# RFD-FHEM/PySignalduino

Hardware: AMD Instinct MI355X
Metric: RF messages/sec demodulated (MU+MS+MC, full protocol bank) (higher is better)
Workload: dtype u8+f64; 1 GPU; mixed MU/MS/MC stream, 1/3 each per rank: MU 256-pulse messages x 129-id MU bank, MS sync+bits x 66-id MS bank (clock x U(0.6,1.4)), MC frames x 12 clockrange ids ('fixed' chain); kind=mixed, corpus=bench, msgs_per_gpu=1000000, batches=3, input_bytes_resident=571611860, parallelism=dp1, grouped=True, streams=one kernel (k_step: MU, then MS, then MC tiles)

## Files before the change

pysignalduino_amd/csrc/sdx_device.h:

```cpp
#pragma once
#include <hip/hip_runtime.h>
#include <stdint.h>

#include "../../include/sdx.h"
#include "../../include/sdx_bank.h"

#define SDX_DEV __device__ __forceinline__

namespace sdx {

constexpr int WAVE = 64;

SDX_DEV double py_round1(double q) {
  if (!(fabs(q) < 562949953421312.0)) return q;
  double f = floor(q * 10.0);
  if (fma(10.0, q, -f) < 0.0) f -= 1.0;
  else if (fma(10.0, q, -(f + 1.0)) >= 0.0) f += 1.0;
  const double r = fma(10.0, q, -(f + 0.5));
  double k;
  if (r > 0.0) k = f + 1.0;
  else if (r < 0.0) k = f;
  else k = (((long long)f & 1) == 0) ? f : f + 1.0;
  double res = k / 10.0;
  if (res == 0.0) res = copysign(0.0, q);
  return res;
}

constexpr int SDX_K_NONE = INT32_MIN;
SDX_DEV int py_round1_k(double q) {
  if (!(fabs(q) < 67108864.0)) return SDX_K_NONE;
  double f = floor(q * 10.0);
  if (fma(10.0, q, -f) < 0.0) f -= 1.0;
  else if (fma(10.0, q, -(f + 1.0)) >= 0.0) f += 1.0;
  const double r = fma(10.0, q, -(f + 0.5));
  double k;
  if (r > 0.0) k = f + 1.0;
  else if (r < 0.0) k = f;
  else k = (((long long)f & 1) == 0) ? f : f + 1.0;
  return (int)k;
}
SDX_DEV void sort10(uint32_t* a) {
#define SDX_CE(i, j)                      \
  {                                       \
    const uint32_t x = a[i], y = a[j];    \
    a[i] = x < y ? x : y;                 \
    a[j] = x < y ? y : x;                 \
  }
  SDX_CE(4, 9) SDX_CE(3, 8) SDX_CE(2, 7) SDX_CE(1, 6) SDX_CE(0, 5) SDX_CE(1, 4) SDX_CE(6, 9) SDX_CE(0, 3)
  SDX_CE(5, 8) SDX_CE(0, 2) SDX_CE(3, 6) SDX_CE(7, 9) SDX_CE(0, 1) SDX_CE(2, 4) SDX_CE(5, 7) SDX_CE(8, 9)
  SDX_CE(1, 2) SDX_CE(4, 6) SDX_CE(7, 8) SDX_CE(3, 5) SDX_CE(2, 5) SDX_CE(6, 8) SDX_CE(1, 3) SDX_CE(4, 7)
  SDX_CE(2, 3) SDX_CE(6, 7) SDX_CE(3, 4) SDX_CE(5, 6) SDX_CE(4, 5)
#undef SDX_CE
}

SDX_DEV bool k_in(int k, int klo, int khi) { return (uint32_t)k - (uint32_t)klo <= (uint32_t)khi - (uint32_t)klo; }

SDX_DEV int lane_id() { return __lane_id(); }
SDX_DEV uint64_t ballot(bool p) { return __ballot(p); }
SDX_DEV int bcast_i(int v, int src) { return __shfl(v, src); }
SDX_DEV uint64_t bcast_u64(uint64_t v, int src) {
  uint32_t lo = __shfl((uint32_t)v, src), hi = __shfl((uint32_t)(v >> 32), src);
  return ((uint64_t)hi << 32) | lo;
}
SDX_DEV int ffs64(uint64_t x) { return __ffsll((unsigned long long)x) - 1; }
SDX_DEV int popc64(uint64_t x) { return __popcll(x); }

SDX_DEV uint64_t bm_window(const uint64_t* bm, int w, int sh, int nw) {
  uint64_t lo = bm[w];
  if (sh == 0) return lo;
  uint64_t hi = (w + 1 < nw) ? bm[w + 1] : 0ull;
  return (lo >> sh) | (hi << (64 - sh));
}

struct PexRes {
  bool found;
  int pos;
  uint64_t tgt;
};

SDX_DEV bool substr_first(const uint64_t* bm, int ws, int nw, uint64_t tgt, int tlen, int minpos, int* pos) {
  for (int w = minpos >> 6; w < nw; ++w) {
    uint64_t acc = ~0ull;
    for (int i = 0; i < tlen && acc; ++i) {
      const int id = (int)((tgt >> (4 * i)) & 15);
      const int sh = i & 63, wo = w + (i >> 6);
      uint64_t v = 0;
      if (wo < nw) v = bm_window(bm + id * ws, wo, sh, nw);
      acc &= v;
    }
    if (w == (minpos >> 6) && (minpos & 63)) acc &= ~0ull << (minpos & 63);
    if (acc) {
      *pos = w * 64 + ffs64(acc);
      return true;
    }
  }
  return false;
}

__device__ __noinline__ PexRes pattern_exists(const sdx_patspec* sp, const int* kq, uint64_t ids, int npat,
                                              const uint64_t* bm, int ws, int nw, int minpos) {
  PexRes res{false, -1, 0};
  const int nu = sp->nuniq, slen = sp->len;
  uint64_t cand[SDX_MAXUNIQ];
  int cnt[SDX_MAXUNIQ];
  long long total = 1;
#pragma unroll
  for (int u = 0; u < SDX_MAXUNIQ; ++u) {
    cand[u] = 0;
    cnt[u] = 1;
    if (u < nu) {
      const double v = sp->uval[u];
      const int klo = sp->klo[u], khi = sp->khi[u];
      double gap[SDX_MAXPAT];
      bool ok[SDX_MAXPAT];
#pragma unroll
      for (int j = 0; j < SDX_MAXPAT; ++j) {
        ok[j] = (j < npat) && k_in(kq[j], klo, khi);
        gap[j] = fabs((double)kq[j] / 10.0 - v);
      }
      int c = 0;
      uint64_t packed = 0;
#pragma unroll
      for (int j = 0; j < SDX_MAXPAT; ++j) {
        if (ok[j]) {
          int rank = 0;
#pragma unroll
          for (int k = 0; k < SDX_MAXPAT; ++k)
            rank += (ok[k] && (gap[k] < gap[j] || (gap[k] == gap[j] && k < j))) ? 1 : 0;
          packed |= (uint64_t)j << (4 * rank);
          ++c;
        }
      }
      cand[u] = packed;
      cnt[u] = c;
      total *= c;
      if (total > 10000) total = 10001;
    }
  }
  if (nu == 0) return res;
  for (int u = 0; u < nu; ++u)
    if (cnt[u] == 0) return res;
  if (total > 10000) return res;
  int digit[SDX_MAXUNIQ];
#pragma unroll
  for (int u = 0; u < SDX_MAXUNIQ; ++u) digit[u] = 0;
  for (long long it = 0; it < total; ++it) {
    uint32_t used = 0, uid = 0;
    bool dup = false;
#pragma unroll
    for (int u = 0; u < SDX_MAXUNIQ; ++u) {
      if (u < nu) {
        const int slot = (int)((cand[u] >> (4 * digit[u])) & 15);
        if (used & (1u << slot)) dup = true;
        used |= 1u << slot;
        uid |= (uint32_t)((ids >> (4 * slot)) & 15) << (4 * u);
      }
    }
    if (!dup) {
      uint64_t tgt = 0;
      for (int i = 0; i < slen; ++i) tgt |= (uint64_t)((uid >> (4 * sp->uidx[i])) & 15) << (4 * i);
      int pos;
      if (substr_first(bm, ws, nw, tgt, slen, minpos, &pos)) {
        res.found = true;
        res.pos = pos;
        res.tgt = tgt;
        return res;
      }
    }
#pragma unroll
    for (int u = SDX_MAXUNIQ - 1; u >= 0; --u) {
      if (u < nu) {
        if (digit[u] + 1 < cnt[u]) {
          digit[u]++;
          break;
        }
        digit[u] = 0;
      }
    }
  }
  return res;
}

SDX_DEV bool match_at(const uint64_t* bm, int ws, int n, uint64_t tgt, int tlen, int x) {
  if (x < 0 || x + tlen > n) return false;
  for (int i = 0; i < tlen; ++i) {
    const int id = (int)((tgt >> (4 * i)) & 15), p = x + i;
    if (!((bm[id * ws + (p >> 6)] >> (p & 63)) & 1ull)) return false;
  }
  return true;
}

SDX_DEV int bval(const uint8_t* b, int a, int e) {
  int v = 0;
  for (int i = a; i < e; ++i) v = (v << 1) | b[i];
  return v;
}
SDX_DEV int first_one(const uint8_t* b, int n) {
  for (int i = 0; i < n; ++i)
    if (b[i] == 1) return i;
  return -1;
}

SDX_DEV int pd_em(const uint8_t* b, int n, uint8_t* o, int* no) {
  int p = -1;
  for (int i = 0; i + 10 <= n; ++i) {
    bool ok = b[i + 9] == 1;
    for (int j = 0; ok && j < 9; ++j) ok = b[i + j] == 0;
    if (ok) { p = i; break; }
  }
  if (p < 0) return 0;
  const uint8_t* s = b + p + 10;
  const int m = n - p - 10;
  if (m != 89) return 0;
  int crc = 0, k = 0;
  for (int c = 0; c + 8 < m; c += 9) {
    if (c < m - 10) {
      for (int j = 7; j >= 0; --j) o[k++] = s[c + j];
      crc ^= bval(s, c, c + 8);
    }
  }
  if (crc != bval(s, m - 8, m)) return 0;
  *no = k;
  return 1;
}

SDX_DEV int pd_revolt(const uint8_t* b, int n, uint8_t* o, int* no) {
  if (n < 96) return 0;
  int sum = 0;
  for (int i = 0; i < 88; i += 8) sum += bval(b, i, i + 8);
  if ((sum & 0xFF) != bval(b, 88, 96)) return 0;
  for (int i = 0; i < 88; ++i) o[i] = b[i];
  *no = 88;
  return 1;
}

SDX_DEV bool groups9_even(const uint8_t* m, int k) {
  for (int g = 0; g < k; g += 9) {
    int par = 0;
    for (int i = g; i < g + 9 && i < k; ++i) par += m[i];
    if (par & 1) return false;
  }
  return true;
}

SDX_DEV int pd_fs20(const uint8_t* b, int n, uint8_t* o, int* no) {
  const int st = first_one(b, n);
  if (st < 0) return 0;
  const uint8_t* m = b + st + 1;
  int k = n - st - 1;
  if (k == 46 || k == 55) --k;
  if (k != 45 && k != 54) return 0;
  int sum = 6;
  for (int g = 0; g < k - 9; g += 9) sum += bval(m, g, g + 8);
  const int chk = bval(m, k - 9, k - 1);
  if (((sum + 6) & 0xFF) == chk) return 0;
  if ((sum & 0xFF) != chk) return 0;
  if (!groups9_even(m, k)) return 0;
  const int nbytes = k / 9;
  int q = 0;
  for (int g = 0; g < nbytes; ++g) {
    if (k == 45 && g == 3) for (int j = 0; j < 8; ++j) o[q++] = 0;
    if (g == nbytes - 1) break;
    for (int j = 0; j < 8; ++j) o[q++] = m[9 * g + j];
  }
  *no = q;
  return 1;
}

SDX_DEV int pd_fht80(const uint8_t* b, int n, uint8_t* o, int* no) {
  const int st = first_one(b, n);
  if (st < 0) return 0;
  const uint8_t* m = b + st + 1;
  int k = n - st - 1;
  if (k == 55) --k;
  if (k != 54) return 0;
  int sum = 12;
  for (int g = 0; g < 45; g += 9) sum += bval(m, g, g + 8);
  const int chk = bval(m, 45, 53);
  if (((sum - 6) & 0xFF) == chk) return 0;
  if ((sum & 0xFF) != chk) return 0;
  if (!groups9_even(m, 54)) return 0;
  int q = 0;
  for (int g = 0; g < 6; ++g)
    for (int j = 0; j < 8; ++j) o[q++] = m[9 * g + j];
  *no = q;
  return 1;
}

SDX_DEV int pd_fht80tf(const uint8_t* b, int n, uint8_t* o, int* no) {
  if (n < 46) return 0;
  const int st = first_one(b, n);
  if (st < 0) return 0;
  const uint8_t* m = b + st + 1;
  const int k = n - st - 1;
  if (k != 45) return 0;
  int sum = 12;
  for (int g = 0; g < 36; g += 9) sum += bval(m, g, g + 8);
  if ((sum & 0xFF) != bval(m, 36, 44)) return 0;
  if (!groups9_even(m, 45)) return 0;
  if (m[9 * 3 + 2] != 0) return 0;
  int q = 0;
  for (int g = 0; g < 4; ++g)
    for (int j = 0; j < 8; ++j) o[q++] = m[9 * g + j];
  *no = q;
  return 1;
}

SDX_DEV int rev_nib(const uint8_t* b, int a, int e) {
  int v = 0;
  for (int i = e - 1; i >= a; --i) v = (v << 1) | b[i];
  return v;
}
SDX_DEV int pd_ws2000(const uint8_t* b, int n, uint8_t* o, int* no) {
  const int st = first_one(b, n);
  if (st < 0) return 0;
  const int dlen = n - st;
  int dlen1 = dlen - dlen % 5;
  const int te = (st + 5 < n) ? st + 5 : n;
  if (te <= st + 1) return -1;
  const int typ = rev_nib(b, st + 1, te);
  if (typ > 7) return 0;
  if (typ == 1 && (dlen == 45 || dlen == 46)) dlen1 += 5;
  const int tab[8] = {35, 50, 35, 50, 70, 40, 40, 85};
  if (tab[typ] != dlen1) return 0;
  if (st > 10) return 0;
  int idx = 0, didx = 0, check = 0, acc = 5;
  while (idx < dlen - 1) {
    if (b[idx + st] != 1) return 0;
    didx = idx + st + 1;
    if (n - didx < 4) return 0;
    const int nib = rev_nib(b, didx, didx + 4);
    if (dlen == 45 || dlen == 46) {
      if (idx <= dlen - 5) check ^= nib;
    } else if (idx <= dlen - 10) {
      check ^= nib;
      acc += nib;
    }
    idx += 5;
  }
  if (check != 0) return 0;
  if (dlen < 45 || dlen > 46) {
    const int e = (didx + 4 < n) ? didx + 4 : n;
    if (e <= didx) return -1;
    if (rev_nib(b, didx, e) != (acc & 0x0F)) return 0;
  }
  const int d = st + 1;
  int q = 0;
  auto rv = [&](int a, int e) {
    for (int i = d + e - 1; i >= d + a; --i)
      if (i < n) o[q++] = b[i];
  };
  rv(5, 9); rv(0, 4); rv(15, 19); rv(10, 14);
  if (typ == 0 || typ == 2) {
    rv(20, 24);
  } else if (typ == 1 || typ == 3 || typ == 4 || typ == 7) {
    rv(25, 29); rv(20, 24); rv(35, 39); rv(30, 34);
    if (typ == 4) { rv(55, 59); rv(50, 54); rv(45, 49); rv(40, 44); }
  }
  *no = q;
  return 1;
}

SDX_DEV int pd_ws7035(const uint8_t* b, int n, uint8_t* o, int* no) {
  if (n < 8) return 0;
  const uint8_t ident[8] = {1, 0, 1, 0, 0, 0, 0, 0};
  for (int i = 0; i < 8; ++i)
    if (b[i] != ident[i]) return 0;
  if (n != 44) return 0;
// ... 148 lines not shown
```

pysignalduino_amd/csrc/sdx_group.hip:

```cpp
#include "sdx_device.h"
#include "sdx_lane.h"

namespace sdx {

SDX_DEV int lanes_below_mask(uint64_t mask) {
  const int l = lane_id();
  return popc64(l ? (mask & ((1ull << l) - 1)) : 0ull);
}
SDX_DEV uint64_t peers8(uint32_t v, bool active) {
  uint64_t peers = ballot(active);
#pragma unroll
  for (int bit = 0; bit < 8; ++bit) {
    const uint64_t bb = ballot(active && ((v >> bit) & 1u));
    peers &= ((v >> bit) & 1u) ? bb : ~bb;
  }
  return peers;
}

constexpr int SIG_PROTOS = 32;
template <int KIND>
SDX_DEV void sig_block(const void* __restrict__ bank, const sdx_pulse_batch& b, uint32_t* __restrict__ key,
                       uint32_t* __restrict__ msg_out, sdx_msg_rec* __restrict__ mrec, const int blk) {
  const BankView bv = bank_view(bank);
  const int i = blk * 256 + threadIdx.x;
  const int ntot = b.sel_dev ? b.n_sel : b.n;
  const bool valid = i < ntot;
  const int msg = valid ? (b.sel_dev ? b.sel_dev[i] : i) : 0;
  int npat = valid ? b.npat_dev[msg] : 0;
  npat = npat > SDX_MAXPAT ? SDX_MAXPAT : npat;
  double val[SDX_MAXPAT];
#pragma unroll
  for (int k = 0; k < SDX_MAXPAT; ++k) val[k] = k < npat ? b.pat_val_dev[msg * SDX_MAXPAT + k] : 0.0;
  int kq[SDX_MAXPAT];
  uint32_t sig = 0;
  auto keys_ok = [&](const SpecV& sv) -> bool {
    bool ok = true;
#pragma unroll
    for (int u = 0; u < SDX_MAXUNIQ; ++u) {
      if (u < sv.nu) {
        bool any = false;
#pragma unroll
        for (int j = 0; j < SDX_MAXPAT; ++j) any |= k_in(kq[j], sv.klo[u], sv.khi[u]);
        ok = ok && any;
      }
    }
    return ok;
  };
  if constexpr (KIND == SDX_KIND_MU) {
    float x10[SDX_MAXPAT];
#pragma unroll
    for (int k = 0; k < SDX_MAXPAT; ++k) x10[k] = (float)(val[k] * 10.0);
    const int nr = (int)bv.hdr->n_mu < SIG_PROTOS ? (int)bv.hdr->n_mu : SIG_PROTOS;
    double last = __builtin_nan("");
    for (int r = 0; r < nr; ++r) {
      const sdx_mu_filt* fr = uniform_ptr(bv.mufilt + r);
      const sdx_mu_proto* rec = uniform_ptr(bv.mu + r);
      const uint32_t ff = cld(&fr->flags);
      bool ok = !(ff & 2u) && (ff & 4u);
      if (ok) {
        const double pclk = cld(&fr->clock);
        if (pclk != last) {
          last = pclk;
          const float inv = 1.0f / (float)pclk;
#pragma unroll
          for (int k = 0; k < SDX_MAXPAT; ++k) {
            const float q = x10[k] * inv;
            kq[k] = (k < npat && fabsf(q) < 1.0e8f) ? (int)rintf(q) : SDX_K_NONE;
          }
        }
        const bool full = (ff & 8u) != 0;
        const int k = (ff & 1u) ? 0 : 1;
        const SpecV sv = full ? spec_full(k == 0 ? &rec->start : &rec->one)
                              : spec_compact(&fr->spec[k], k == 0 ? cld(&fr->start_upk) : (uint64_t)cld(&fr->spec[k].upk));
        if (sv.slen) ok = ok && keys_ok(sv);
      }
      sig |= (uint32_t)ok << (31 - r);
    }
  } else {
    const int cp = valid ? b.cp_slot_dev[msg] : -1;
    double clock = 0.0;
#pragma unroll
    for (int k = 0; k < SDX_MAXPAT; ++k)
      if (k == cp) clock = fabs(val[k]);
    const bool gate = valid && b.ms_ok_dev[msg] && cp >= 0 && cp < npat && clock != 0.0;
    const float inv = clock != 0.0 ? (float)(10.0 / clock) : 0.0f;
#pragma unroll
    for (int k = 0; k < SDX_MAXPAT; ++k) {
      const float q = (float)val[k] * inv;
      kq[k] = (gate && k < npat && fabsf(q) < 1.0e8f) ? (int)rintf(q) : SDX_K_NONE;
    }
    const int nr = (int)bv.hdr->n_ms < SIG_PROTOS ? (int)bv.hdr->n_ms : SIG_PROTOS;
    for (int r = 0; r < nr; ++r) {
      const sdx_ms_filt* fr = uniform_ptr(bv.msfilt + r);
      const sdx_ms_proto* rec = uniform_ptr(bv.ms + r);
      const uint32_t ff = cld(&fr->flags);
      bool ok = gate && !(ff & 2u);
      const double pclk = cld(&fr->pclock);
      if (ok && pclk > 0.0) ok = !(fabs(pclk - clock) > clock * 0.3);
      if (ok) {
        const bool full = (ff & 8u) != 0;
        const SpecV sv = full ? spec_full(&rec->key[0]) : spec_compact(&fr->spec[0], cld(&fr->sync_upk));
        if (sv.slen) ok = ok && keys_ok(sv);
      }
      sig |= (uint32_t)ok << (31 - r);
    }
  }
  if (valid && mrec) {
    const int64_t off = b.offsets_dev[msg];
    const int32_t len = b.len_dev ? b.len_dev[msg] : (int32_t)(b.offsets_dev[msg + 1] - off);
    uint32_t id[4] = {0, 0, 0, 0};
#pragma unroll
    for (int k = 0; k < SDX_MAXPAT; ++k) id[k >> 2] |= (uint32_t)b.pat_id_dev[msg * SDX_MAXPAT + k] << (8 * (k & 3));
    const uint32_t w3 = (uint32_t)(valid ? b.npat_dev[msg] : 0) |
                        ((uint32_t)(uint8_t)(KIND == SDX_KIND_MS ? b.cp_slot_dev[msg] : -1) << 8) |
                        ((uint32_t)(KIND == SDX_KIND_MS ? b.ms_ok_dev[msg] : 0) << 16);
    uint4* d = reinterpret_cast<uint4*>(mrec + msg);
    d[0] = make_uint4((uint32_t)off, (uint32_t)((uint64_t)off >> 32), (uint32_t)len, w3);
    d[1] = make_uint4(id[0], id[1], id[2], 0u);
#pragma unroll
    for (int h = 0; h < SDX_MAXPAT / 2; ++h) {
      const uint64_t a = (uint64_t)__double_as_longlong(val[2 * h]), c = (uint64_t)__double_as_longlong(val[2 * h + 1]);
      d[2 + h] = make_uint4((uint32_t)a, (uint32_t)(a >> 32), (uint32_t)c, (uint32_t)(c >> 32));
    }
    d[7] = make_uint4(0u, 0u, 0u, 0u);
  }
  if (valid) {
    const int64_t o = b.offsets_dev[msg];
    const int len = b.len_dev ? b.len_dev[msg] : (int)(b.offsets_dev[msg + 1] - o);
    const uint32_t ms_key = (len > 128 ? 0x80000000u : 0u) | (sig >> 1);
    key[i] = KIND == SDX_KIND_MU ? ~sig : ms_key;
    msg_out[i] = (uint32_t)msg;
  }
}

template <int KIND>
__global__ __launch_bounds__(256) void k_sig(const void* __restrict__ bank, sdx_pulse_batch b, uint32_t* __restrict__ key,
                                             uint32_t* __restrict__ msg_out, sdx_msg_rec* __restrict__ mrec) {
  sig_block<KIND>(bank, b, key, msg_out, mrec, (int)blockIdx.x);
}

struct SigSide {
  sdx_pulse_batch b;
  uint32_t* key;
  uint32_t* msg;
  sdx_msg_rec* mrec;
};
__global__ __launch_bounds__(256) void k_sig2(const void* __restrict__ bank, SigSide mu, SigSide ms, int g_mu) {
  if ((int)blockIdx.x < g_mu)
    sig_block<SDX_KIND_MU>(bank, mu.b, mu.key, mu.msg, mu.mrec, (int)blockIdx.x);
  else
    sig_block<SDX_KIND_MS>(bank, ms.b, ms.key, ms.msg, ms.mrec, (int)blockIdx.x - g_mu);
}

constexpr int RS_T = 512, RS_ROUNDS = 4, RS_PART = RS_T * RS_ROUNDS;
constexpr int RS_PASSES = 4;

SDX_DEV void rs_hist(const uint32_t* __restrict__ key, int n, int np, int d, uint32_t* __restrict__ hist, const int p,
                     uint32_t* c) {
  const int tid = threadIdx.x;
  if (tid < 256) c[tid] = 0;
  __syncthreads();
  for (int r = 0; r < RS_ROUNDS; ++r) {
    const int e = p * RS_PART + r * RS_T + tid;
    const bool valid = e < n;
    const uint32_t dig = valid ? (key[e] >> (8 * d)) & 255u : 0u;
    const uint64_t peers = peers8(dig, valid);
    if (valid && lane_id() == ffs64(peers)) atomicAdd(&c[dig], (uint32_t)popc64(peers));
  }
  __syncthreads();
  if (tid < 256) hist[(size_t)tid * np + p] = c[tid];
}
__global__ __launch_bounds__(RS_T) void k_rs_hist(const uint32_t* __restrict__ key, int n, int np, int d,
                                                  uint32_t* __restrict__ hist) {
  __shared__ uint32_t c[256];
  rs_hist(key, n, np, d, hist, (int)blockIdx.x, c);
}

SDX_DEV void rs_scan_rows(uint32_t* __restrict__ hist, int np, uint32_t* __restrict__ tot, const int blk) {
  const int row = blk * 4 + (threadIdx.x >> 6), lane = threadIdx.x & 63;
  uint32_t* h = hist + (size_t)row * np;
  uint32_t run = 0;
  for (int b0 = 0; b0 < np; b0 += 64) {
    const int x = b0 + lane;
    const uint32_t v = x < np ? h[x] : 0u;
    uint32_t incl = v;
#pragma unroll
    for (int o = 1; o < 64; o <<= 1) {
      const uint32_t y = __shfl_up(incl, o);
      if (lane >= o) incl += y;
    }
    if (x < np) h[x] = run + incl - v;
    run += __shfl(incl, 63);
  }
  if (lane == 0) tot[row] = run;
}
__global__ __launch_bounds__(256) void k_rs_scan_rows(uint32_t* __restrict__ hist, int np, uint32_t* __restrict__ tot) {
  rs_scan_rows(hist, np, tot, (int)blockIdx.x);
}

SDX_DEV void rs_scatter(const uint32_t* __restrict__ kin, const uint32_t* __restrict__ vin, int n, int np, int d,
                        const uint32_t* __restrict__ hist, const uint32_t* __restrict__ tot, uint32_t* __restrict__ kout,
                        uint32_t* __restrict__ vout, const int p, uint32_t* run, uint32_t (*wc)[256]) {
  const int tid = threadIdx.x, wave = tid >> 6;
  const uint32_t t = tid < 256 ? tot[tid] : 0u;
  if (tid < 256) run[tid] = t;
  __syncthreads();
  for (int o = 1; o < 256; o <<= 1) {
    const uint32_t y = (tid < 256 && tid >= o) ? run[tid - o] : 0u;
    __syncthreads();
    if (tid < 256) run[tid] += y;
    __syncthreads();
  }
  if (tid < 256) run[tid] = run[tid] - t + hist[(size_t)tid * np + p];
  for (int r = 0; r < RS_ROUNDS; ++r) {
    const int e = p * RS_PART + r * RS_T + tid;
    const bool valid = e < n;
    const uint32_t k = valid ? kin[e] : 0u;
    const uint32_t v = valid ? vin[e] : 0u;
    const uint32_t dig = (k >> (8 * d)) & 255u;
    for (int x = tid; x < RS_T / 64 * 256; x += RS_T) (&wc[0][0])[x] = 0;
    __syncthreads();
    const uint64_t peers = peers8(dig, valid);
    if (valid && lane_id() == ffs64(peers)) wc[wave][dig] = (uint32_t)popc64(peers);
    __syncthreads();
    if (valid) {
      uint32_t pos = run[dig] + (uint32_t)lanes_below_mask(peers);
      for (int w = 0; w < wave; ++w) pos += wc[w][dig];
      kout[pos] = k;
      vout[pos] = v;
    }
    __syncthreads();
    if (tid < 256) {
      uint32_t add = 0;
#pragma unroll
      for (int w = 0; w < RS_T / 64; ++w) add += wc[w][tid];
      run[tid] += add;
    }
    __syncthreads();
  }
}
__global__ __launch_bounds__(RS_T) void k_rs_scatter(const uint32_t* __restrict__ kin, const uint32_t* __restrict__ vin,
                                                     int n, int np, int d, const uint32_t* __restrict__ hist,
                                                     const uint32_t* __restrict__ tot, uint32_t* __restrict__ kout,
                                                     uint32_t* __restrict__ vout) {
  __shared__ uint32_t run[256];
  __shared__ uint32_t wc[RS_T / 64][256];
  rs_scatter(kin, vin, n, np, d, hist, tot, kout, vout, (int)blockIdx.x, run, wc);
}

struct RsPass {
  const uint32_t* kin;
  const uint32_t* vin;
  uint32_t* kout;
  uint32_t* vout;
  uint32_t* hist;
  uint32_t* tot;
  int n, np;
};
__global__ __launch_bounds__(RS_T) void k_rs_hist2(RsPass a, RsPass b, int d) {
  __shared__ uint32_t c[256];
  const bool second = (int)blockIdx.x >= a.np;
  const RsPass& x = second ? b : a;
  rs_hist(x.kin, x.n, x.np, d, x.hist, second ? (int)blockIdx.x - a.np : (int)blockIdx.x, c);
}
__global__ __launch_bounds__(256) void k_rs_scan_rows2(RsPass a, RsPass b) {
  const bool second = blockIdx.x >= 256 / 4;
  const RsPass& x = second ? b : a;
  rs_scan_rows(x.hist, x.np, x.tot, (int)blockIdx.x - (second ? 256 / 4 : 0));
}
__global__ __launch_bounds__(RS_T) void k_rs_scatter2(RsPass a, RsPass b, int d) {
  __shared__ uint32_t run[256];
  __shared__ uint32_t wc[RS_T / 64][256];
  const bool second = (int)blockIdx.x >= a.np;
  const RsPass& x = second ? b : a;
  rs_scatter(x.kin, x.vin, x.n, x.np, d, x.hist, x.tot, x.kout, x.vout,
             second ? (int)blockIdx.x - a.np : (int)blockIdx.x, run, wc);
}

constexpr size_t align256(size_t x) { return (x + 255) & ~(size_t)255; }

size_t group_bytes(int n) {
  if (n <= 0) return 0;
  const size_t np = (size_t)(n + RS_PART - 1) / RS_PART;
  return 4 * align256(4 * (size_t)n) + align256(4 * 256 * np) + align256(4 * 256);
}

bool group_messages(const void* bank_dev, int kind, const sdx_pulse_batch& b, int32_t* order, sdx_msg_rec* mrec,
                    uint8_t* work, size_t bytes, hipStream_t st) {
  const int n = b.sel_dev ? b.n_sel : b.n;
  const size_t need = group_bytes(n);
  if (!need || bytes < need) return false;
  const int np = (n + RS_PART - 1) / RS_PART;
  const size_t a = align256(4 * (size_t)n);
  uint32_t* k0 = reinterpret_cast<uint32_t*>(work);
  uint32_t* v0 = reinterpret_cast<uint32_t*>(work + a);
  uint32_t* k1 = reinterpret_cast<uint32_t*>(work + 2 * a);
  uint32_t* v1 = reinterpret_cast<uint32_t*>(work + 3 * a);
  uint32_t* hist = reinterpret_cast<uint32_t*>(work + 4 * a);
  uint32_t* tot = reinterpret_cast<uint32_t*>(work + 4 * a + align256(4 * 256 * (size_t)np));
  const int grid = (n + 255) / 256;
  if (kind == SDX_KIND_MU)
    hipLaunchKernelGGL((k_sig<SDX_KIND_MU>), dim3(grid), dim3(256), 0, st, bank_dev, b, k0, v0, mrec);
  else
    hipLaunchKernelGGL((k_sig<SDX_KIND_MS>), dim3(grid), dim3(256), 0, st, bank_dev, b, k0, v0, mrec);
  for (int pi = 0; pi < RS_PASSES; ++pi) {
    const int d = 4 - RS_PASSES + pi;
    const bool even = (pi & 1) == 0;
    uint32_t* kin = even ? k0 : k1;
    uint32_t* vout = pi == RS_PASSES - 1 ? reinterpret_cast<uint32_t*>(order) : (even ? v1 : v0);
    hipLaunchKernelGGL(k_rs_hist, dim3(np), dim3(RS_T), 0, st, kin, n, np, d, hist);
    hipLaunchKernelGGL(k_rs_scan_rows, dim3(256 / 4), dim3(256), 0, st, hist, np, tot);
    hipLaunchKernelGGL(k_rs_scatter, dim3(np), dim3(RS_T), 0, st, kin, even ? v0 : v1, n, np, d, hist, tot,
                       even ? k1 : k0, vout);
  }
  return hipGetLastError() == hipSuccess;
}

bool group_messages2(const void* bank_dev, const sdx_pulse_batch& bmu, int32_t* omu, sdx_msg_rec* rmu, uint8_t* wmu,
                     size_t cmu, const sdx_pulse_batch& bms, int32_t* oms, sdx_msg_rec* rms, uint8_t* wms, size_t cms,
                     hipStream_t st) {
  const int nmu = bmu.sel_dev ? bmu.n_sel : bmu.n, nms = bms.sel_dev ? bms.n_sel : bms.n;
  if (nmu <= 0 || nms <= 0 || cmu < group_bytes(nmu) || cms < group_bytes(nms)) return false;
  struct Side {
    uint32_t *k0, *v0, *k1, *v1, *hist, *tot;
    int n, np;
  };
  auto side = [](uint8_t* work, int n) {
    Side x;
    const size_t a = align256(4 * (size_t)n);
    x.n = n;
    x.np = (n + RS_PART - 1) / RS_PART;
    x.k0 = reinterpret_cast<uint32_t*>(work);
    x.v0 = reinterpret_cast<uint32_t*>(work + a);
    x.k1 = reinterpret_cast<uint32_t*>(work + 2 * a);
    x.v1 = reinterpret_cast<uint32_t*>(work + 3 * a);
    x.hist = reinterpret_cast<uint32_t*>(work + 4 * a);
    x.tot = reinterpret_cast<uint32_t*>(work + 4 * a + align256(4 * 256 * (size_t)x.np));
    return x;
  };
  const Side A = side(wmu, nmu), B = side(wms, nms);
  const int gmu = (nmu + 255) / 256, gms = (nms + 255) / 256;
  hipLaunchKernelGGL(k_sig2, dim3(gmu + gms), dim3(256), 0, st, bank_dev, SigSide{bmu, A.k0, A.v0, rmu},
                     SigSide{bms, B.k0, B.v0, rms}, gmu);
  for (int pi = 0; pi < RS_PASSES; ++pi) {
    const int d = 4 - RS_PASSES + pi;
    const bool even = (pi & 1) == 0;
    const bool last = pi == RS_PASSES - 1;
    auto pass = [&](const Side& x, int32_t* order) {
      return RsPass{even ? x.k0 : x.k1, even ? x.v0 : x.v1, even ? x.k1 : x.k0,
                    last ? reinterpret_cast<uint32_t*>(order) : (even ? x.v1 : x.v0), x.hist, x.tot, x.n, x.np};
    };
    const RsPass pa = pass(A, omu), pb = pass(B, oms);
    hipLaunchKernelGGL(k_rs_hist2, dim3(A.np + B.np), dim3(RS_T), 0, st, pa, pb, d);
    hipLaunchKernelGGL(k_rs_scan_rows2, dim3(2 * (256 / 4)), dim3(256), 0, st, pa, pb);
    hipLaunchKernelGGL(k_rs_scatter2, dim3(A.np + B.np), dim3(RS_T), 0, st, pa, pb, d);
  }
  return hipGetLastError() == hipSuccess;
}

}
```

pysignalduino_amd/csrc/sdx_tile.h:

```cpp
#pragma once
#include "sdx_device.h"
#include "sdx_lane.h"

#include <type_traits>

#ifdef SDX_WGTIME
__device__ unsigned long long g_wgt[2 * 65536];
#endif
#ifdef SDX_PROF
__device__ unsigned long long g_prof[32];
__device__ unsigned long long g_gprof[2][128];
#define PROF_T(v) unsigned long long v = __builtin_amdgcn_s_memtime()
#define PROF_ADD(slot, v)                                                                   \
  do {                                                                                      \
    if (__lane_id() == 0) L.prof[wave][slot] += (unsigned)(__builtin_amdgcn_s_memtime() - (v)); \
  } while (0)
#define PROF_CNT(slot, x)                                                                   \
  do {                                                                                      \
    if (__lane_id() == 0) L.prof[wave][slot] += (unsigned)(x);                              \
  } while (0)
#define PROF_ADDD(slot, v)                                                                  \
  do {                                                                                      \
    if (__lane_id() == __ffsll((unsigned long long)__builtin_amdgcn_read_exec()) - 1)       \
      L.prof[wave][slot] += (unsigned)(__builtin_amdgcn_s_memtime() - (v));                 \
  } while (0)
#define PROF_CNTL(slot) atomicAdd(&L.prof[wave][slot], 1u)
#else
#define PROF_T(v)
#define PROF_ADD(slot, v)
#define PROF_ADDD(slot, v)
#define PROF_CNT(slot, x)
#define PROF_CNTL(slot)
#endif

namespace sdx {

constexpr int POOL_REC = 640;
constexpr int POOL_HEAP = 16384;
constexpr int POOL_REC_MS = 256;
constexpr int POOL_HEAP_MS = 8192;

struct StageRec {
  uint32_t off;
  uint16_t len, proto;
  uint32_t bitlen;
  uint8_t msg, wave;
  uint16_t rank;
};
constexpr uint32_t STAGE_NIB = 0x80000000u;
SDX_DEV uint32_t stage_bitlen(int bitlen, int hex_digits, int pre_len) {
  return (hex_digits >= 0 && hex_digits < 32768 && pre_len <= 255 && (uint32_t)bitlen < 65536u)
             ? (STAGE_NIB | ((uint32_t)hex_digits << 16) | (uint32_t)bitlen)
             : (uint32_t)bitlen;
}

struct MuItem {
  uint32_t st_lo, st_hi;
  uint16_t u0, u1, u2;
  uint16_t idx, p;
  uint8_t mi, fmask;
};
constexpr int QCAP = 128;
constexpr int LANE_WAVES = 8;

struct MsItem {
  uint32_t k0_lo, k0_hi;
  uint16_t k1, k2, k3;
  uint16_t start;
  uint16_t p;
  uint8_t mi, fmask;
};
constexpr int MS_SURV_CAP = 1024;
constexpr int MS_DESC_LDS = 96;
struct MsDesc {
  int32_t lir_min, lir_max, pad, pre_off, post_off;
  uint16_t pre_len, post_len;
  uint8_t width, klen[4], recon, postdemo, res;
};
static_assert(sizeof(MsDesc) == 32, "MsDesc layout");

struct MuMatch {
  uint16_t q, k;
  uint16_t u0, u1, u2;
  uint16_t p;
  uint8_t mi;
  uint8_t flags;
  uint8_t j;
};
constexpr int MATCH_CAP = 768;

constexpr uint32_t SPILL_M = 2048, SPILL_R = 2048, SPILL_H = 49152;
constexpr uint32_t SPILL_OFF_R = SPILL_M * 16, SPILL_OFF_H = SPILL_OFF_R + SPILL_R * 16;
constexpr uint32_t SPILL_BYTES = SPILL_OFF_H + SPILL_H;
constexpr uint32_t SPILL_NONE = 0xFFFFFFFFu, SPILL_PENDING = 0xFFFFFFFEu, SPILL_FULL = 0xFFFFFFFDu;
constexpr uint32_t HEAP_SPILLED = 0x80000000u;
constexpr uint8_t REC_HOLE = 0xFF;
static_assert(sizeof(MuMatch) == 16, "MuMatch spill layout");

template <int NW, int TM, int LM>
struct TileLds {
  static constexpr int WS = NW;
  static constexpr int MSTRIDE = 10 * NW + 1;
  static constexpr int NBITS = 64 * NW + 64;
  struct Wave {
    uint64_t umask[3][NW];
    uint64_t uany[NW];
    uint64_t smask[NW];
    uint64_t stream[NW + 18];
    uint8_t bits[NBITS];
    uint8_t bits2[NBITS];
  };
  uint64_t bm[TM * MSTRIDE];
  uint64_t pairs[TM][2];
  int32_t nlen[TM];
  uint32_t raise_key[TM];
  uint32_t digit_ok[TM];
  uint32_t cnt[TM];
  uint32_t rec_base, heap_base, tile_bad, tot_rec;
  uint32_t mbase[TM];
  struct WaveScratch4 {
    Wave w[4];
  };
  struct NoScratch {};
  typename std::conditional<LM != 0, NoScratch, WaveScratch4>::type wa;
  static constexpr int PREC = LM == 1 ? 512 : (NW <= 4 ? POOL_REC_MS * (TM > 64 ? 2 : 1) : POOL_REC);
  static constexpr int PHEAP =
      LM == 1 ? 10240 : (NW <= 4 ? POOL_HEAP_MS * (TM > 64 ? 2 : 1) : POOL_HEAP);
  static constexpr int SCAP = TM > 64 ? MS_SURV_CAP + MS_SURV_CAP / 4 : MS_SURV_CAP;
  static constexpr int NHALF = (LM == 2 && TM > 64) ? 2 : 1;
  static_assert(TM <= 64 * NHALF, "one lane per message of a half");
  StageRec rec[PREC];
  alignas(16) uint8_t heap[PHEAP];
  unsigned long long pool_ctr;
  uint32_t spill_base, sp_rec, sp_heap;
  int ovf, next_p[NHALF];
  int mm_states, nmatch;
  MuMatch mlist[LM == 1 ? MATCH_CAP : 1];
  alignas(16) sdx_mu_desc desc[LM == 1 ? SDX_MUDESC_LDS : 1];
  union alignas(16) {
    MuItem q[LM == 1 ? LANE_WAVES : 1][LM == 1 ? QCAP : 1];
    uint8_t mmtab[LM == 1 ? SDX_MMTAB_LDS : 16];
  } u;
  MsItem slist[LM == 2 ? SCAP : 1];
  int nsurv;
  MsDesc msdesc[LM == 2 ? MS_DESC_LDS : 1];
#ifdef SDX_PROF
  unsigned int prof[LM != 0 ? LANE_WAVES : 4][28];
#endif
};

SDX_DEV void wave_sync() {
  __builtin_amdgcn_fence(__ATOMIC_SEQ_CST, "wavefront");
  __builtin_amdgcn_wave_barrier();
}

template <int G>
SDX_DEV uint32_t group_or(uint32_t v) {
  static_assert(G == 8 || G == 16, "a half row or a row of 16 lanes");
  v |= (uint32_t)__builtin_amdgcn_update_dpp(0, (int)v, 0xB1, 0xF, 0xF, true);
  v |= (uint32_t)__builtin_amdgcn_update_dpp(0, (int)v, 0x4E, 0xF, 0xF, true);
  v |= (uint32_t)__builtin_amdgcn_update_dpp(0, (int)v, 0x141, 0xF, 0xF, true);
  if constexpr (G == 16) v |= (uint32_t)__builtin_amdgcn_update_dpp(0, (int)v, 0x140, 0xF, 0xF, true);
  return v;
}

SDX_DEV int lanes_below(uint64_t mask) {
  const int l = lane_id();
  return popc64(l ? (mask & ((1ull << l) - 1)) : 0ull);
}

template <class T>
SDX_DEV int pool_alloc(T& L, int total, int* rec_slot) {
  int h = -1, r = -1;
  if (lane_id() == 0) {
    const unsigned long long o = atomicAdd(&L.pool_ctr, ((unsigned long long)total << 32) | 1ull);
    r = (int)(uint32_t)o;
    h = (int)(o >> 32);
    if (r >= T::PREC || h + total > T::PHEAP) {
      L.ovf = 1;
      h = -1;
    }
  }
  h = bcast_i(h, 0);
  *rec_slot = bcast_i(r, 0);
  return h;
}

template <class T>
SDX_DEV void pool_commit(T& L, int slot, int wave, int msg_local, int proto, int off, int total, int bitlen) {
  if (lane_id() == 0) {
    StageRec r;
    r.off = (uint32_t)off;
    r.len = (uint16_t)total;
    r.proto = (uint16_t)proto;
    r.bitlen = (uint32_t)bitlen;
    r.msg = (uint8_t)msg_local;
    r.wave = (uint8_t)wave;
    r.rank = (uint16_t)atomicAdd(&L.cnt[msg_local], 1u);
    L.rec[slot] = r;
  }
  wave_sync();
}

template <class T>
SDX_DEV uint32_t spill_region(T& L, const sdx_out& out) {
  uint32_t b = __hip_atomic_load(&L.spill_base, __ATOMIC_RELAXED, __HIP_MEMORY_SCOPE_WORKGROUP);
  if (b >= SPILL_PENDING) {
    const int leader = ffs64(ballot(true));
    if (lane_id() == leader) {
      uint32_t cur = atomicCAS(&L.spill_base, SPILL_NONE, SPILL_PENDING);
      if (cur == SPILL_NONE) {
        const uint32_t idx = atomicAdd(&out.cursor_dev[3], 1u);
        const uint64_t o = (uint64_t)idx * SPILL_BYTES;
        cur = (out.work_dev && o + SPILL_BYTES <= out.work_cap) ? (uint32_t)o : SPILL_FULL;
        __hip_atomic_store(&L.spill_base, cur, __ATOMIC_RELAXED, __HIP_MEMORY_SCOPE_WORKGROUP);
      }
      while (cur == SPILL_PENDING) cur = __hip_atomic_load(&L.spill_base, __ATOMIC_RELAXED, __HIP_MEMORY_SCOPE_WORKGROUP);
      b = cur;
    }
    b = (uint32_t)__shfl((int)b, leader);
  }
  if (b == SPILL_FULL || !out.work_dev || (uint64_t)b + SPILL_BYTES > out.work_cap) return SPILL_NONE;
  return b;
}

struct PoolSlot {
  StageRec* rec;
  uint8_t* heap;
  uint32_t off;
};
template <class T>
SDX_DEV bool pool_take(T& L, const sdx_out& out, int span, PoolSlot* ps) {
  const unsigned long long o = atomicAdd(&L.pool_ctr, ((unsigned long long)span << 32) | 1ull);
  const int slot = (int)(uint32_t)o, off = (int)(o >> 32);
  if (slot < T::PREC && off + span <= T::PHEAP) {
    ps->rec = &L.rec[slot];
    ps->heap = L.heap + off;
    ps->off = (uint32_t)off;
    return true;
  }
  if (slot < T::PREC) L.rec[slot].msg = REC_HOLE;
  const uint32_t base = spill_region(L, out);
  const uint32_t rs = atomicAdd(&L.sp_rec, 1u), hs = atomicAdd(&L.sp_heap, (uint32_t)span);
  if (base == SPILL_NONE || rs >= SPILL_R || hs + (uint32_t)span > SPILL_H) {
    L.ovf = 1;
    return false;
  }
  uint8_t* reg = out.work_dev + base;
  ps->rec = reinterpret_cast<StageRec*>(reg + SPILL_OFF_R) + rs;
  ps->heap = reg + SPILL_OFF_H + hs;
  ps->off = HEAP_SPILLED | hs;
  return true;
}

SDX_DEV void copy_str(uint8_t* dst, const uint8_t* src, int n) {
  for (int i = lane_id(); i < n; i += WAVE) dst[i] = src[i];
}

SDX_DEV int any_float(const uint8_t* bits, int nb) {
  bool f = false;
  for (int i = lane_id(); i < nb; i += WAVE) f |= bits[i] == 2;
  return ballot(f) != 0;
}

SDX_DEV int hex_digits(const uint8_t* bits, int nb, uint8_t* dst, int strip_zero) {
  const int nd = (nb + 3) >> 2;
  int skip = 0;
  if (strip_zero) {
    skip = nd;
    for (int d0 = 0; d0 < nd; d0 += WAVE) {
      const int d = d0 + lane_id();
      int v = 0;
      if (d < nd) {
        const int e = nb - 4 * (nd - 1 - d), a = (e - 4 > 0) ? e - 4 : 0;
        for (int i = a; i < e; ++i) v = (v << 1) | bits[i];
      }
      const uint64_t nz = ballot(d < nd && v != 0);
      if (nz) {
        skip = d0 + ffs64(nz);
        break;
      }
    }
  }
  for (int d = skip + lane_id(); d < nd; d += WAVE) {
    const int e = nb - 4 * (nd - 1 - d), a = (e - 4 > 0) ? e - 4 : 0;
    int v = 0;
    for (int i = a; i < e; ++i) v = (v << 1) | bits[i];
    dst[d - skip] = (uint8_t)(v < 10 ? '0' + v : 'A' + v - 10);
  }
  return nd - skip;
}

template <class T>
SDX_DEV void raise_msg(T& L, int msg_local, int proto, int kind) {
  if (lane_id() == 0) atomicMin(&L.raise_key[msg_local], ((uint32_t)proto << 8) | (uint32_t)kind);
  wave_sync();
}

template <int NW, int TM, int LM>
SDX_DEV void finish_mu(TileLds<NW, TM, LM>& L, int wave, const BankView& bv, const sdx_mu_proto* rec, int p, int s,
                       int nb) {
  auto& W = L.wa.w[wave];
  uint8_t* buf = W.bits;
  PROF_T(t_pd);
  if (cld(&rec->postdemo) != SDX_PD_NONE && !any_float(buf, nb)) {
    int rc = 0, no = 0;
    if (lane_id() == 0) rc = run_postdemo(cld(&rec->postdemo), buf, nb, W.bits2, &no);
    rc = bcast_i(rc, 0);
    no = bcast_i(no, 0);
    wave_sync();
    if (rc == 0) return;
    if (rc == 1) {
      buf = W.bits2;
      nb = no;
    }
  }
  PROF_ADD(7, t_pd);
  PROF_T(t_fmt);
  const int pad = cld(&rec->pad_bits);
  int nbp = nb;
  nbp = (nbp + pad - 1) / pad * pad;
  for (int i = nb + lane_id(); i < nbp; i += WAVE) buf[i] = 0;
  wave_sync();
  const bool isf = any_float(buf, nbp);
  int dlen;
  if (cld(&rec->dispatch_bin)) dlen = nbp;
  else if (isf) {
    if (cld(&rec->remove_zero)) {
      raise_msg(L, s, p, SDX_RAISE_ATTRIBUTE);
      return;
    }
    dlen = 4;
  } else {
    dlen = -2;
  }
  const int nd = (nbp + 3) >> 2;
  int skip = 0;
  if (dlen == -2) {
    if (cld(&rec->remove_zero)) {
      skip = nd;
      for (int d0 = 0; d0 < nd; d0 += WAVE) {
        const int d = d0 + lane_id();
        int v = 0;
        if (d < nd) {
          const int e = nbp - 4 * (nd - 1 - d), a = (e - 4 > 0) ? e - 4 : 0;
          for (int i = a; i < e; ++i) v = (v << 1) | buf[i];
        }
        const uint64_t nz = ballot(d < nd && v != 0);
        if (nz) {
          skip = d0 + ffs64(nz);
          break;
        }
      }
    }
    dlen = nd - skip;
  }
  auto dchar = [&](int d) -> uint8_t {
    if (cld(&rec->dispatch_bin)) return buf[d] == 2 ? 'F' : (uint8_t)('0' + buf[d]);
    if (isf) return (uint8_t)"None"[d];
    const int dd = d + skip, e = nbp - 4 * (nd - 1 - dd), a = (e - 4 > 0) ? e - 4 : 0;
    int v = 0;
    for (int i = a; i < e; ++i) v = (v << 1) | buf[i];
    return (uint8_t)(v < 10 ? '0' + v : 'A' + v - 10);
  };
  if (cld(&rec->mm_dfa) >= 0) {
    int ok = 0;
    if (lane_id() == 0) {
      const sdx_dfa D = bv.dfa[cld(&rec->mm_dfa)];
      const uint8_t* t256 = bv.t256 + D.t256_off;
      const uint8_t* fl = bv.dflags + D.flags_off;
      int st = cld(&rec->mm_pre_state);
      const int tot = dlen + cld(&rec->post_len);
      int i = 0;
      for (; i < tot; ++i) {
        const uint8_t f = fl[st];
        if (f & 5) break;
        const uint8_t c = i < dlen ? dchar(i) : bv.str[cld(&rec->post_off) + i - dlen];
        st = t256[st * 256 + c];
      }
      const uint8_t f = fl[st];
      ok = (f & 1) ? 1 : ((f & 4) ? 0 : ((i == tot && (f & 2)) ? 1 : 0));
    }
    PROF_ADD(9, t_fmt);
    if (!bcast_i(ok, 0)) return;
  }
  PROF_T(t_wr);
  const int total = cld(&rec->pre_len) + dlen + cld(&rec->post_len);
  int slot;
  const int off = pool_alloc(L, total, &slot);
  if (off < 0) return;
  uint8_t* dst = L.heap + off;
  copy_str(dst, bv.str + cld(&rec->pre_off), cld(&rec->pre_len));
  for (int d = lane_id(); d < dlen; d += WAVE) dst[cld(&rec->pre_len) + d] = dchar(d);
  copy_str(dst + cld(&rec->pre_len) + dlen, bv.str + cld(&rec->post_off), cld(&rec->post_len));
  pool_commit(L, slot, wave, s, p, off, total, (int)stage_bitlen(nbp, isf ? -1 : dlen, cld(&rec->pre_len)));
  PROF_ADD(8, t_wr);
  PROF_CNT(20, 1);
}

template <int NW, int TM, int LM>
SDX_DEV void decode_mu(TileLds<NW, TM, LM>& L, int wave, const BankView& bv, const sdx_mu_proto* rec, int p, int s,
                       int idx, uint64_t st_tgt, uint64_t ut0, uint64_t ut1, uint64_t ut2, int fmask) {
  using T = TileLds<NW, TM, LM>;
  auto& W = L.wa.w[wave];
  const int lane = lane_id();
  const uint64_t* bm = &L.bm[s * T::MSTRIDE];
  const int n = L.nlen[s], nw = (n + 63) >> 6;
  const int Lw = cld(&rec->width);
  const int lenS = cld(&rec->has_start) ? (int)cld(&rec->start.len) : 0;
  const uint64_t ut[3] = {ut0, ut1, ut2};
  const uint8_t SYM[3] = {1, 0, 2};
  PROF_T(t_setup);
  PROF_CNT(21, 1);
  uint64_t uni[3] = {0, 0, 0};
  uint8_t usym[3] = {0, 0, 0};
  int nu = 0;
  for (int k = 0; k < 3; ++k) {
    if (!((fmask >> k) & 1)) continue;
    int j = 0;
    for (; j < nu; ++j)
      if (uni[j] == ut[k]) break;
    if (j == nu) uni[nu++] = ut[k];
    usym[j] = SYM[k];
  }
  uint64_t ek[3] = {0, 0, 0};
  uint8_t esym[3] = {0, 0, 0};
  int ne = 0;
  if (cld(&rec->recon) && Lw > 1) {
    const uint64_t msk = (Lw - 1 >= 16) ? ~0ull : ((1ull << (4 * (Lw - 1))) - 1);
    for (int k = 0; k < 3; ++k) {
      if (!((fmask >> k) & 1)) continue;
      const uint64_t key = ut[k] & msk;
      int j = 0;
      for (; j < ne; ++j)
        if (ek[j] == key) break;
      if (j == ne) {
        ek[ne] = key;
        esym[ne] = SYM[k];
        ++ne;
      }
    }
  }
  if (lane < nw) {
    uint64_t any = 0;
    for (int j = 0; j < nu; ++j) {
      uint64_t m = ~0ull;
      for (int i = 0; i < Lw; ++i) {
        const int id = (int)((uni[j] >> (4 * i)) & 15), wo = lane + (i >> 6);
        m &= (wo < nw) ? bm_window(bm + id * T::WS, wo, i & 63, nw) : 0ull;
      }
      W.umask[j][lane] = m;
      any |= m;
    }
    W.uany[lane] = any;
    uint64_t sm = ~0ull;
    for (int i = 0; i < lenS; ++i) {
      const int id = (int)((st_tgt >> (4 * i)) & 15), wo = lane + (i >> 6);
      sm &= (wo < nw) ? bm_window(bm + id * T::WS, wo, i & 63, nw) : 0ull;
// ... 1650 lines not shown
```

Baseline: 700.9 million msgs/s.

## Specialize signature loop for narrow patterns and restructure radix sort scan/scatter

The signature computation is templated on the pattern count, so a wave where no message has more than 8 patterns runs a narrower loop with fewer key comparisons. The radix sort histogram and scatter now load each thread's keys up front in a wave-contiguous layout. Per-wave digit counts are accumulated with wave-level syncs instead of repeated block barriers per round. The 256-bucket total scan and the row scan handle 4 elements per lane with shuffles, replacing the barrier-heavy shared-memory scan. This cuts block-level synchronisation and redundant work in the grouping stage, at the cost of two template instantiations and more registers.

```diff
diff --git a/pysignalduino_amd/csrc/sdx_device.h b/pysignalduino_amd/csrc/sdx_device.h
--- a/pysignalduino_amd/csrc/sdx_device.h
+++ b/pysignalduino_amd/csrc/sdx_device.h
@@ -64,6 +64,10 @@
 }
 SDX_DEV int ffs64(uint64_t x) { return __ffsll((unsigned long long)x) - 1; }
 SDX_DEV int popc64(uint64_t x) { return __popcll(x); }
+SDX_DEV void wave_sync() {
+  __builtin_amdgcn_fence(__ATOMIC_SEQ_CST, "wavefront");
+  __builtin_amdgcn_wave_barrier();
+}
 
 SDX_DEV uint64_t bm_window(const uint64_t* bm, int w, int sh, int nw) {
   uint64_t lo = bm[w];
diff --git a/pysignalduino_amd/csrc/sdx_group.hip b/pysignalduino_amd/csrc/sdx_group.hip
--- a/pysignalduino_amd/csrc/sdx_group.hip
+++ b/pysignalduino_amd/csrc/sdx_group.hip
@@ -18,20 +18,11 @@
 }
 
 constexpr int SIG_PROTOS = 32;
-template <int KIND>
-SDX_DEV void sig_block(const void* __restrict__ bank, const sdx_pulse_batch& b, uint32_t* __restrict__ key,
-                       uint32_t* __restrict__ msg_out, sdx_msg_rec* __restrict__ mrec, const int blk) {
-  const BankView bv = bank_view(bank);
-  const int i = blk * 256 + threadIdx.x;
-  const int ntot = b.sel_dev ? b.n_sel : b.n;
-  const bool valid = i < ntot;
-  const int msg = valid ? (b.sel_dev ? b.sel_dev[i] : i) : 0;
-  int npat = valid ? b.npat_dev[msg] : 0;
-  npat = npat > SDX_MAXPAT ? SDX_MAXPAT : npat;
-  double val[SDX_MAXPAT];
-#pragma unroll
-  for (int k = 0; k < SDX_MAXPAT; ++k) val[k] = k < npat ? b.pat_val_dev[msg * SDX_MAXPAT + k] : 0.0;
-  int kq[SDX_MAXPAT];
+constexpr int SIG_NARROW = 8;
+template <int KIND, int NP>
+SDX_DEV uint32_t sig_bits(const BankView& bv, const sdx_pulse_batch& b, const double* val, const int npat,
+                          const bool valid, const int msg) {
+  int kq[NP];
   uint32_t sig = 0;
   auto keys_ok = [&](const SpecV& sv) -> bool {
     bool ok = true;
@@ -40,32 +31,33 @@
       if (u < sv.nu) {
         bool any = false;
 #pragma unroll
-        for (int j = 0; j < SDX_MAXPAT; ++j) any |= k_in(kq[j], sv.klo[u], sv.khi[u]);
+        for (int j = 0; j < NP; ++j) any |= k_in(kq[j], sv.klo[u], sv.khi[u]);
         ok = ok && any;
       }
     }
     return ok;
   };
   if constexpr (KIND == SDX_KIND_MU) {
-    float x10[SDX_MAXPAT];
-#pragma unroll
-    for (int k = 0; k < SDX_MAXPAT; ++k) x10[k] = (float)(val[k] * 10.0);
+    float x10[NP];
+#pragma unroll
+    for (int k = 0; k < NP; ++k) x10[k] = (float)(val[k] * 10.0);
     const int nr = (int)bv.hdr->n_mu < SIG_PROTOS ? (int)bv.hdr->n_mu : SIG_PROTOS;
     double last = __builtin_nan("");
     for (int r = 0; r < nr; ++r) {
       const sdx_mu_filt* fr = uniform_ptr(bv.mufilt + r);
       const sdx_mu_proto* rec = uniform_ptr(bv.mu + r);
       const uint32_t ff = cld(&fr->flags);
+      const double pclk = cld(&fr->clock);
       bool ok = !(ff & 2u) && (ff & 4u);
       if (ok) {
-        const double pclk = cld(&fr->clock);
         if (pclk != last) {
           last = pclk;
           const float inv = 1.0f / (float)pclk;
 #pragma unroll
-          for (int k = 0; k < SDX_MAXPAT; ++k) {
+          for (int k = 0; k < NP; ++k) {
             const float q = x10[k] * inv;
-            kq[k] = (k < npat && fabsf(q) < 1.0e8f) ? (int)rintf(q) : SDX_K_NONE;
+            const bool in = (k < npat) & (fabsf(q) < 1.0e8f);
+            kq[k] = in ? (int)rintf(in ? q : 0.0f) : SDX_K_NONE;
           }
         }
         const bool full = (ff & 8u) != 0;
@@ -85,9 +77,10 @@
     const bool gate = valid && b.ms_ok_dev[msg] && cp >= 0 && cp < npat && clock != 0.0;
     const float inv = clock != 0.0 ? (float)(10.0 / clock) : 0.0f;
 #pragma unroll
-    for (int k = 0; k < SDX_MAXPAT; ++k) {
+    for (int k = 0; k < NP; ++k) {
       const float q = (float)val[k] * inv;
-      kq[k] = (gate && k < npat && fabsf(q) < 1.0e8f) ? (int)rintf(q) : SDX_K_NONE;
+      const bool in = gate & (k < npat) & (fabsf(q) < 1.0e8f);
+      kq[k] = in ? (int)rintf(in ? q : 0.0f) : SDX_K_NONE;
     }
     const int nr = (int)bv.hdr->n_ms < SIG_PROTOS ? (int)bv.hdr->n_ms : SIG_PROTOS;
     for (int r = 0; r < nr; ++r) {
@@ -105,6 +98,24 @@
       sig |= (uint32_t)ok << (31 - r);
     }
   }
+  return sig;
+}
+
+template <int KIND>
+SDX_DEV void sig_block(const void* __restrict__ bank, const sdx_pulse_batch& b, uint32_t* __restrict__ key,
+                       uint32_t* __restrict__ msg_out, sdx_msg_rec* __restrict__ mrec, const int blk) {
+  const BankView bv = bank_view(bank);
+  const int i = blk * 256 + threadIdx.x;
+  const int ntot = b.sel_dev ? b.n_sel : b.n;
+  const bool valid = i < ntot;
+  const int msg = valid ? (b.sel_dev ? b.sel_dev[i] : i) : 0;
+  int npat = valid ? b.npat_dev[msg] : 0;
+  npat = npat > SDX_MAXPAT ? SDX_MAXPAT : npat;
+  double val[SDX_MAXPAT];
+#pragma unroll
+  for (int k = 0; k < SDX_MAXPAT; ++k) val[k] = k < npat ? b.pat_val_dev[msg * SDX_MAXPAT + k] : 0.0;
+  const uint32_t sig = ballot(npat > SIG_NARROW) ? sig_bits<KIND, SDX_MAXPAT>(bv, b, val, npat, valid, msg)
+                                                 : sig_bits<KIND, SIG_NARROW>(bv, b, val, npat, valid, msg);
   if (valid && mrec) {
     const int64_t off = b.offsets_dev[msg];
     const int32_t len = b.len_dev ? b.len_dev[msg] : (int32_t)(b.offsets_dev[msg + 1] - off);
@@ -152,18 +163,22 @@
     sig_block<SDX_KIND_MS>(bank, ms.b, ms.key, ms.msg, ms.mrec, (int)blockIdx.x - g_mu);
 }
 
-constexpr int RS_T = 512, RS_ROUNDS = 4, RS_PART = RS_T * RS_ROUNDS;
+constexpr int RS_T = 512, RS_WAVES = RS_T / 64, RS_ROUNDS = 4, RS_WAVE = 64 * RS_ROUNDS, RS_PART = RS_T * RS_ROUNDS;
 constexpr int RS_PASSES = 4;
 
 SDX_DEV void rs_hist(const uint32_t* __restrict__ key, int n, int np, int d, uint32_t* __restrict__ hist, const int p,
                      uint32_t* c) {
   const int tid = threadIdx.x;
+  const int e0 = p * RS_PART + (tid >> 6) * RS_WAVE + (tid & 63);
+  uint32_t k[RS_ROUNDS];
+#pragma unroll
+  for (int s = 0; s < RS_ROUNDS; ++s) k[s] = e0 + 64 * s < n ? key[e0 + 64 * s] : 0u;
   if (tid < 256) c[tid] = 0;
   __syncthreads();
-  for (int r = 0; r < RS_ROUNDS; ++r) {
-    const int e = p * RS_PART + r * RS_T + tid;
-    const bool valid = e < n;
-    const uint32_t dig = valid ? (key[e] >> (8 * d)) & 255u : 0u;
+#pragma unroll
+  for (int s = 0; s < RS_ROUNDS; ++s) {
+    const bool valid = e0 + 64 * s < n;
+    const uint32_t dig = (k[s] >> (8 * d)) & 255u;
     const uint64_t peers = peers8(dig, valid);
     if (valid && lane_id() == ffs64(peers)) atomicAdd(&c[dig], (uint32_t)popc64(peers));
   }
@@ -180,16 +195,26 @@
   const int row = blk * 4 + (threadIdx.x >> 6), lane = threadIdx.x & 63;
   uint32_t* h = hist + (size_t)row * np;
   uint32_t run = 0;
-  for (int b0 = 0; b0 < np; b0 += 64) {
-    const int x = b0 + lane;
-    const uint32_t v = x < np ? h[x] : 0u;
-    uint32_t incl = v;
+  for (int b0 = 0; b0 < np; b0 += 256) {
+    const int x0 = b0 + 4 * lane;
+    uint32_t v[4], sum = 0;
+#pragma unroll
+    for (int c = 0; c < 4; ++c) {
+      v[c] = x0 + c < np ? h[x0 + c] : 0u;
+      sum += v[c];
+    }
+    uint32_t incl = sum;
 #pragma unroll
     for (int o = 1; o < 64; o <<= 1) {
       const uint32_t y = __shfl_up(incl, o);
       if (lane >= o) incl += y;
     }
-    if (x < np) h[x] = run + incl - v;
+    uint32_t b = run + incl - sum;
+#pragma unroll
+    for (int c = 0; c < 4; ++c) {
+      if (x0 + c < np) h[x0 + c] = b;
+      b += v[c];
+    }
     run += __shfl(incl, 63);
   }
   if (lane == 0) tot[row] = run;
@@ -200,52 +225,79 @@
 
 SDX_DEV void rs_scatter(const uint32_t* __restrict__ kin, const uint32_t* __restrict__ vin, int n, int np, int d,
                         const uint32_t* __restrict__ hist, const uint32_t* __restrict__ tot, uint32_t* __restrict__ kout,
-                        uint32_t* __restrict__ vout, const int p, uint32_t* run, uint32_t (*wc)[256]) {
-  const int tid = threadIdx.x, wave = tid >> 6;
-  const uint32_t t = tid < 256 ? tot[tid] : 0u;
-  if (tid < 256) run[tid] = t;
+                        uint32_t* __restrict__ vout, const int p, uint32_t* base, uint32_t (*wc)[256]) {
+  const int tid = threadIdx.x, wave = tid >> 6, lane = tid & 63;
+  const int e0 = p * RS_PART + wave * RS_WAVE + lane;
+  uint32_t k[RS_ROUNDS], v[RS_ROUNDS];
+#pragma unroll
+  for (int s = 0; s < RS_ROUNDS; ++s) {
+    const bool valid = e0 + 64 * s < n;
+    k[s] = valid ? kin[e0 + 64 * s] : 0u;
+    v[s] = valid ? vin[e0 + 64 * s] : 0u;
+  }
+  const uint32_t row = tid < 256 ? hist[(size_t)tid * np + p] : 0u;
+#pragma unroll
+  for (int x = 0; x < 4; ++x) wc[wave][64 * x + lane] = 0;
+  if (wave == RS_WAVES - 1) {
+    uint32_t t[4], sum = 0;
+#pragma unroll
+    for (int x = 0; x < 4; ++x) {
+      t[x] = tot[4 * lane + x];
+      sum += t[x];
+    }
+    uint32_t incl = sum;
+#pragma unroll
+    for (int o = 1; o < 64; o <<= 1) {
+      const uint32_t y = __shfl_up(incl, o);
+      if (lane >= o) incl += y;
+    }
+    uint32_t b = incl - sum;
+#pragma unroll
+    for (int x = 0; x < 4; ++x) {
+      base[4 * lane + x] = b;
+      b += t[x];
+    }
+  }
+  wave_sync();
+  uint64_t peers[RS_ROUNDS];
+  uint32_t before[RS_ROUNDS];
+#pragma unroll
+  for (int s = 0; s < RS_ROUNDS; ++s) {
+    const bool valid = e0 + 64 * s < n;
+    const uint32_t dig = (k[s] >> (8 * d)) & 255u;
+    peers[s] = peers8(dig, valid);
+    before[s] = wc[wave][dig];
+    wave_sync();
+    if (valid && lane == ffs64(peers[s])) wc[wave][dig] = before[s] + (uint32_t)popc64(peers[s]);
+    wave_sync();
+  }
   __syncthreads();
-  for (int o = 1; o < 256; o <<= 1) {
-    const uint32_t y = (tid < 256 && tid >= o) ? run[tid - o] : 0u;
-    __syncthreads();
-    if (tid < 256) run[tid] += y;
-    __syncthreads();
-  }
-  if (tid < 256) run[tid] = run[tid] - t + hist[(size_t)tid * np + p];
-  for (int r = 0; r < RS_ROUNDS; ++r) {
-    const int e = p * RS_PART + r * RS_T + tid;
-    const bool valid = e < n;
-    const uint32_t k = valid ? kin[e] : 0u;
-    const uint32_t v = valid ? vin[e] : 0u;
-    const uint32_t dig = (k >> (8 * d)) & 255u;
-    for (int x = tid; x < RS_T / 64 * 256; x += RS_T) (&wc[0][0])[x] = 0;
-    __syncthreads();
-    const uint64_t peers = peers8(dig, valid);
-    if (valid && lane_id() == ffs64(peers)) wc[wave][dig] = (uint32_t)popc64(peers);
-    __syncthreads();
-    if (valid) {
-      uint32_t pos = run[dig] + (uint32_t)lanes_below_mask(peers);
-      for (int w = 0; w < wave; ++w) pos += wc[w][dig];
-      kout[pos] = k;
-      vout[pos] = v;
-    }
-    __syncthreads();
-    if (tid < 256) {
-      uint32_t add = 0;
-#pragma unroll
-      for (int w = 0; w < RS_T / 64; ++w) add += wc[w][tid];
-      run[tid] += add;
-    }
-    __syncthreads();
+  if (tid < 256) {
+    uint32_t run = base[tid] + row;
+#pragma unroll
+    for (int w = 0; w < RS_WAVES; ++w) {
+      const uint32_t c = wc[w][tid];
+      wc[w][tid] = run;
+      run += c;
+    }
+  }
+  __syncthreads();
+#pragma unroll
+  for (int s = 0; s < RS_ROUNDS; ++s) {
+    if (e0 + 64 * s < n) {
+      const uint32_t pos = wc[wave][(k[s] >> (8 * d)) & 255u] + before[s] + (uint32_t)lanes_below_mask(peers[s]);
+      kout[pos] = k[s];
+      vout[pos] = v[s];
+    }
   }
 }
 __global__ __launch_bounds__(RS_T) void k_rs_scatter(const uint32_t* __restrict__ kin, const uint32_t* __restrict__ vin,
                                                      int n, int np, int d, const uint32_t* __restrict__ hist,
                                                      const uint32_t* __restrict__ tot, uint32_t* __restrict__ kout,
                                                      uint32_t* __restrict__ vout) {
-  __shared__ uint32_t run[256];
-  __shared__ uint32_t wc[RS_T / 64][256];
-  rs_scatter(kin, vin, n, np, d, hist, tot, kout, vout, (int)blockIdx.x, run, wc);
+  __shared__ uint32_t base[256];
+  __shared__ uint32_t wc[RS_WAVES][256];
+  rs_scatter(kin, vin, n, np, d, hist, tot, kout, vout, (int)blockIdx.x, base, wc);
 }
 
 struct RsPass {
@@ -269,12 +321,12 @@
   rs_scan_rows(x.hist, x.np, x.tot, (int)blockIdx.x - (second ? 256 / 4 : 0));
 }
 __global__ __launch_bounds__(RS_T) void k_rs_scatter2(RsPass a, RsPass b, int d) {
-  __shared__ uint32_t run[256];
-  __shared__ uint32_t wc[RS_T / 64][256];
+  __shared__ uint32_t base[256];
+  __shared__ uint32_t wc[RS_WAVES][256];
   const bool second = (int)blockIdx.x >= a.np;
   const RsPass& x = second ? b : a;
   rs_scatter(x.kin, x.vin, x.n, x.np, d, x.hist, x.tot, x.kout, x.vout,
-             second ? (int)blockIdx.x - a.np : (int)blockIdx.x, run, wc);
+             second ? (int)blockIdx.x - a.np : (int)blockIdx.x, base, wc);
 }
 
 constexpr size_t align256(size_t x) { return (x + 255) & ~(size_t)255; }
diff --git a/pysignalduino_amd/csrc/sdx_tile.h b/pysignalduino_amd/csrc/sdx_tile.h
--- a/pysignalduino_amd/csrc/sdx_tile.h
+++ b/pysignalduino_amd/csrc/sdx_tile.h
@@ -149,11 +149,6 @@
 #endif
 };
 
-SDX_DEV void wave_sync() {
-  __builtin_amdgcn_fence(__ATOMIC_SEQ_CST, "wavefront");
-  __builtin_amdgcn_wave_barrier();
-}
-
 template <int G>
 SDX_DEV uint32_t group_or(uint32_t v) {
   static_assert(G == 8 || G == 16, "a half row or a row of 16 lanes");
```

Result: faster. 708.0 million msgs/s (median of 6 runs) (+1.0%).
